# wooginawunan/multi-modal-uncertainty

Hardware: AMD Instinct MI355X
Metric: image+text samples/sec/node, MMBT Food-101 bs=256 seq=512; ECE/NLL parity (higher is better)
Workload: dtype bf16

## Files before the change

include/mmu.h:

```cpp
#ifndef MMU_H
#define MMU_H
#include <stdint.h>

#ifdef __cplusplus
extern "C" {
#endif

typedef void* mmu_stream_t;

enum { MMU_BF16 = 0, MMU_F32 = 1 };

#define MMU_ABI_VERSION 4
int mmu_version(void);
const char* mmu_last_error(void);

int mmu_set_seed_offset(const uint64_t* dev_counter);

int mmu_set_deterministic(int on);
int mmu_get_deterministic(void);

enum {
  MMU_EPI_STORE = 0,
  MMU_EPI_BIAS_GELU = 1,
  MMU_EPI_BIAS_DROP_RES = 2,
// ... 15 lines not shown
  int64_t ldx, aux_bstride;
  float* colsum;
  int64_t colsum_bstride;
  float drop_p;
  uint64_t seed;
  float* workspace;
  int64_t workspace_floats;
  const float* res_ln_mean;
  const float* res_ln_rstd;
  const float* res_ln_w;
  const float* res_ln_b;
  int64_t res_ln_bstride;
  const void* bn_x;
  const uint8_t* bn_mask;
  const float* bn_mean;
  const uint8_t* res_mask;
} mmu_epilogue;

int mmu_gemm(const void* A, int64_t lda, int a_kmajor,
             const void* B, int64_t ldb, int b_kmajor,
             void* C, int64_t ldc, int c_dtype,
             int64_t M, int64_t N, int64_t K,
             int64_t batch, int64_t strideA, int64_t strideB, int64_t strideC,
             const mmu_epilogue* epi, mmu_stream_t stream);

int mmu_gemm_rows(const void* A, int64_t lda, int a_kmajor,
                  const void* B, int64_t ldb, int b_kmajor,
                  void* C, int64_t ldc, int c_dtype,
                  int64_t M, int64_t N, int64_t K,
                  int64_t batch, int64_t strideA, int64_t strideB, int64_t strideC,
                  const mmu_epilogue* epi, int64_t drop_row_step, int64_t drop_row_offset,
                  mmu_stream_t stream);

int mmu_colsum_reduce(const float* partial, int64_t parts, int64_t N, float* out,
                      int accumulate, mmu_stream_t stream);
int mmu_colsum_reduce_multi(int n, const float* const* partial, const int64_t* parts, float* const* out, int64_t N,
                            int accumulate, mmu_stream_t stream);
int mmu_colsum_bf16(const void* X, int64_t M, int64_t N, int64_t ldx, float* partial,
                    float* out, int accumulate, mmu_stream_t stream);

int mmu_transpose_bf16_batched(const int64_t* jobs, int n_jobs, int64_t max_rows, int64_t max_cols,
                               mmu_stream_t stream);

int mmu_attention_fwd(const void* QKV, int64_t ld_qkv, const float* keymask,
                      void* O, int64_t ld_o, float* LSE,
                      int64_t batch, int64_t L, int64_t heads,
                      float drop_p, uint64_t seed, uint64_t* dropmask, mmu_stream_t stream);
int mmu_attention_bwd(const void* QKV, int64_t ld_qkv, const float* keymask,
                      const void* O, int64_t ld_o, const void* dO, int64_t ld_do,
                      const float* LSE, float* delta, void* dQKV, int64_t ld_dqkv,
                      int64_t batch, int64_t L, int64_t heads,
                      float drop_p, uint64_t seed, const uint64_t* dropmask, float* dbias_parts,
                      mmu_stream_t stream);

int mmu_attention_row0_fwd(const void* QKV, int64_t ld_qkv, const float* keymask,
                           void* O, int64_t ld_o, float* LSE,
                           int64_t batch, int64_t L, int64_t heads,
                           float drop_p, uint64_t seed, uint64_t* dropmask, mmu_stream_t stream);
int mmu_attention_row0_bwd(const void* QKV, int64_t ld_qkv, const float* keymask,
                           const void* O, int64_t ld_o, const void* dO, int64_t ld_do,
                           const float* LSE, void* dQKV, int64_t ld_dqkv,
                           int64_t batch, int64_t L, int64_t heads,
                           float drop_p, const uint64_t* dropmask, float* dbias_sums,
                           mmu_stream_t stream);

int mmu_layernorm_fwd(const void* X, const float* w, const float* b, void* Y,
// ... 184 lines not shown
```

multi-modal-uncertainty_amd/csrc/capi.hip:

```cpp
#include <stdarg.h>
#include <stdio.h>
#include <atomic>
#include <map>
#include <tuple>
#include <mutex>
#include <string>
#include <vector>
#include "mmu_internal.h"
#include <cstdlib>
#include <cmath>

using namespace mmu;

static thread_local std::string g_err;

namespace mmu {
const uint64_t* g_seed_off = nullptr;

static std::atomic<int> g_det{-1};
bool deterministic() {
  int v = g_det.load(std::memory_order_relaxed);
  if (v < 0) {
    const char* e = getenv("MMU_DETERMINISTIC");
    int want = (e && atoi(e) == 1) ? 1 : 0;
// ... 43 lines not shown

std::pair<hipEvent_t, hipEvent_t> take_events() {
  std::lock_guard<std::mutex> lk(g_t.mu);
  std::pair<hipEvent_t, hipEvent_t> ev;
  if (!g_t.pool.empty()) {
    ev = g_t.pool.back();
    g_t.pool.pop_back();
  } else {
    (void)hipEventCreate(&ev.first);
    (void)hipEventCreate(&ev.second);
  }
  return ev;
}
constexpr int64_t TAIL_WS_FLOATS = 8ll << 20;
float* tail_workspace(int64_t floats, hipStream_t s, int slot = 0) {
  static std::mutex mu;
  static std::map<std::tuple<int, hipStream_t, int>, float*> bufs;
  if (floats > TAIL_WS_FLOATS) return nullptr;
  int dev = 0;
  if (hipGetDevice(&dev) != hipSuccess) return nullptr;
  std::lock_guard<std::mutex> lk(mu);
  auto it = bufs.find({dev, s, slot});
  if (it != bufs.end()) return it->second;
  hipStreamCaptureStatus st = hipStreamCaptureStatusNone;
  if (hipStreamIsCapturing(s, &st) != hipSuccess || st != hipStreamCaptureStatusNone) return nullptr;
  void* b = nullptr;
  if (hipMalloc(&b, sizeof(float) * TAIL_WS_FLOATS) != hipSuccess) {
    (void)hipGetLastError();
    return nullptr;
  }
  bufs[{dev, s, slot}] = (float*)b;
  return (float*)b;
}
}

extern "C" {

int mmu_version(void) { return MMU_ABI_VERSION; }
const char* mmu_last_error(void) { return g_err.c_str(); }

int mmu_timing_enable(int on) {
  std::lock_guard<std::mutex> lk(g_t.mu);
  g_t.on = on != 0;
  for (auto& e : g_t.used) g_t.pool.push_back(e);
  g_t.used.clear();
  g_t.flops.clear();
  return 0;
}

int mmu_timing_pause(int paused) {
  std::lock_guard<std::mutex> lk(g_t.mu);
  g_t.paused = paused != 0;
  return 0;
}

int mmu_timing_read(double* total_ms, int64_t* launches, double* flops) {
  std::lock_guard<std::mutex> lk(g_t.mu);
  double tot = 0.0, fl = 0.0;
  for (size_t i = 0; i < g_t.used.size(); ++i) {
    (void)hipEventSynchronize(g_t.used[i].second);
    float ms = 0.f;
    if (hipEventElapsedTime(&ms, g_t.used[i].first, g_t.used[i].second) != hipSuccess) return fail("timing: elapsed");
    tot += ms;
    fl += g_t.flops[i];
  }
  *total_ms = tot;
  *launches = (int64_t)g_t.used.size();
  *flops = fl;
  return 0;
}

static int gemm_impl(const void* A, int64_t lda, int a_kmajor, const void* B, int64_t ldb, int b_kmajor, void* C,
                     int64_t ldc, int c_dtype, int64_t M, int64_t N, int64_t K, int64_t batch, int64_t strideA,
                     int64_t strideB, int64_t strideC, const mmu_epilogue* epi, int64_t drop_row_step,
                     int64_t drop_row_off, mmu_stream_t stream) {
  if (!A || !B || !C) return fail("mmu_gemm: null operand");
  if (M <= 0 || N <= 0 || K <= 0 || batch <= 0) return fail("mmu_gemm: bad shape M=%ld N=%ld K=%ld", M, N, K);
  if (N % 128) return fail("mmu_gemm: N=%ld must be a multiple of 128", N);
  if ((a_kmajor || b_kmajor) && K % 64) return fail("mmu_gemm: K=%ld must be a multiple of 64 for a K-major operand", K);
  if (!a_kmajor && M % 128) return fail("mmu_gemm: M=%ld must be a multiple of 128 when A is M-major", M);
  if ((lda % 8) || (ldb % 8) || (ldc % 4)) return fail("mmu_gemm: leading dims must be 16-B aligned");
  if (c_dtype != MMU_BF16 && c_dtype != MMU_F32) return fail("mmu_gemm: bad c_dtype");
  GemmParams p{};
  p.A = (const bf16*)A; p.B = (const bf16*)B; p.C = C;
  p.lda = lda; p.ldb = ldb; p.ldc = ldc; p.M = M; p.N = N; p.K = K;
  p.sA = strideA; p.sB = strideB; p.sC = strideC;
  p.drop_ldn = N * drop_row_step; p.drop_base = N * drop_row_off;
  const int64_t a_span = 2 * (a_kmajor ? (M + 256) * lda : (K + 64) * lda);
  const int64_t b_span = 2 * (b_kmajor ? (N + 256) * ldb : (K + 64) * ldb);
  const bool big = M >= 256 && N >= 256 && a_span < (1ll << 32) - 4096 && b_span < (1ll << 32) - 4096;
  const int tile = big ? 256 : 128;
  p.tiles_m = (int)((M + tile - 1) / tile);
  p.tiles_n = (int)((N + tile - 1) / tile);
  int kind = MMU_EPI_STORE;
  if (epi) kind = epi->kind;
  p.group_m = p.tiles_n <= 3 ? 1 : ((b_kmajor && kind != MMU_EPI_DGELU) ? 8 : 2);
  if (epi) {
    kind = epi->kind;
    p.accumulate = epi->accumulate;
    p.bias = epi->bias; p.bias_bstride = epi->bias_bstride;
    p.residual = epi->residual; p.ldr = epi->ldr; p.res_bstride = epi->res_bstride;
    p.aux = epi->aux; p.ldx = epi->ldx; p.aux_bstride = epi->aux_bstride;
    p.colsum = epi->colsum; p.colsum_bstride = epi->colsum_bstride;
    p.drop_p = epi->drop_p; p.seed = epi->seed; p.seed_off = g_seed_off;
    p.res_ln_mean = epi->res_ln_mean; p.res_ln_rstd = epi->res_ln_rstd;
    p.res_ln_w = epi->res_ln_w; p.res_ln_b = epi->res_ln_b; p.res_ln_bstride = epi->res_ln_bstride;
    p.bn_x = (const bf16*)epi->bn_x; p.bn_mask = epi->bn_mask; p.bn_mean = epi->bn_mean;
    p.res_mask = epi->res_mask;
  }
  p.kind = kind;
  if (kind < 0 || kind > MMU_EPI_ADD_RES_BNB) return fail("mmu_gemm: bad epilogue kind %d", kind);
  if ((kind == MMU_EPI_STORE_BNB || kind == MMU_EPI_ADD_RES_BNB) &&
      (!p.colsum || !p.bn_x || !p.bn_mean || batch != 1 || !a_kmajor || b_kmajor || p.accumulate || p.bias ||
       ldc != N || c_dtype != MMU_BF16))
    return fail("mmu_gemm: *_BNB needs the table (colsum), bn_x, bn_mean, batch 1, K-major A, N-major B, "
                "bf16 C with ldc == N, no bias / accumulate");
  if (kind == MMU_EPI_STORE_STATS && (!p.colsum || batch != 1 || !a_kmajor || !b_kmajor || p.accumulate))
    return fail("mmu_gemm: STORE_STATS needs the stats table (colsum), batch 1, K-major A and B, no accumulate");
  if (kind != MMU_EPI_STORE && kind != MMU_EPI_BIAS_DROP_RES && c_dtype != MMU_BF16)
    return fail("mmu_gemm: fused epilogues other than BIAS_DROP_RES write bf16");
  if (kind == MMU_EPI_BIAS_DROP_RES && c_dtype == MMU_F32 && (ldc % 4 || (epi && epi->ldr % 4)))
    return fail("mmu_gemm: f32 hidden-stream epilogue needs 16-B aligned rows");
  {
    const int nln = !!p.res_ln_mean + !!p.res_ln_rstd + !!p.res_ln_w + !!p.res_ln_b;
    if (nln && (nln != 4 || kind != MMU_EPI_BIAS_DROP_RES || c_dtype != MMU_F32))
      return fail("mmu_gemm: res_ln_* (all four) only with BIAS_DROP_RES into an f32 C");
  }
  if (kind == MMU_EPI_DGELU && !p.aux) return fail("mmu_gemm: DGELU epilogue needs aux");
  if ((kind == MMU_EPI_BIAS_DROP_RES || kind == MMU_EPI_ADD_RES || kind == MMU_EPI_ADD_RES_BNB) && !p.residual)
// ... 25 lines not shown
    if (p.res_ln_w && (off16(p.res_ln_w) || off16(p.res_ln_b) || (bat && p.res_ln_bstride % 4)))
      return fail("mmu_gemm: res_ln_w, res_ln_b and res_ln_bstride must keep 16-B alignment");
    if (p.res_ln_w && (((uintptr_t)p.res_ln_mean | (uintptr_t)p.res_ln_rstd) & 3))
      return fail("mmu_gemm: res_ln_mean / res_ln_rstd must be 4-B aligned");
    const bool table = kind == MMU_EPI_STORE_STATS || kind == MMU_EPI_STORE_BNB || kind == MMU_EPI_ADD_RES_BNB;
    if (table && off16(p.colsum)) return fail("mmu_gemm: the float2 table (colsum) must be 16-B aligned");
    if (!table && p.colsum && ((uintptr_t)p.colsum & 3)) return fail("mmu_gemm: colsum must be 4-B aligned");
    if (epi && epi->workspace && off16(epi->workspace))
      return fail("mmu_gemm: the split-K workspace must be 16-B aligned (float4 slabs)");
    if ((kind == MMU_EPI_STORE_BNB || kind == MMU_EPI_ADD_RES_BNB) && (off16(p.bn_x) || off16(p.bn_mean)))
      return fail("mmu_gemm: bn_x and bn_mean must be 16-B aligned");
  }
  p.splitk = 1;
  p.kchunk = K;
  if (kind == MMU_EPI_STORE && c_dtype == MMU_F32 && !p.bias && !p.colsum && epi && epi->workspace && K >= 1024) {
    const int64_t tiles = (int64_t)p.tiles_m * p.tiles_n * batch;
    const int64_t max_split = 64, min_k = K >= 32768 ? 1024 : 256;
    int64_t want = (640 + tiles - 1) / tiles;
    if (want > K / min_k) want = K / min_k;
    if (want > max_split) want = max_split;
    const int64_t cap = epi->workspace_floats / (batch * M * N);
    if (want > cap) want = cap;
    if (want >= 2) {
      int64_t chunk = (K + want - 1) / want;
      chunk = (chunk + 63) / 64 * 64;
      p.kchunk = chunk;
      p.splitk = (int)((K + chunk - 1) / chunk);
      p.ws = epi->workspace;
    }
  }
  const char* wide_env = getenv("MMU_GEMM_WIDE");
  const char* wide_min_env = getenv("MMU_GEMM_WIDE_MIN_TILES");
  const int wide_mode = wide_env ? atoi(wide_env) : 1;
  const int64_t wide_min = wide_min_env ? (int64_t)atoll(wide_min_env) : (int64_t)1024;
  const bool tail_kind = kind == MMU_EPI_STORE || kind == MMU_EPI_BIAS_GELU || kind == MMU_EPI_BIAS_DROP_RES ||
                         kind == MMU_EPI_DGELU || kind == MMU_EPI_ADD_RES;
  const bool wide_kind = tail_kind && kind != MMU_EPI_DGELU;
  const bool wide = (wide_mode == 2 ? tail_kind : wide_mode == 1 && wide_kind && N >= 2304) && big && a_kmajor &&
                    b_kmajor && N % 384 == 0 && p.splitk == 1 &&
                    2 * (M + 256) * lda < (1ll << 32) - 4096 && 2 * (N + 384) * ldb < (1ll << 32) - 4096 &&
                    (M + 255) / 256 * (N / 384) * batch >= wide_min;
  if (wide) {
    p.tiles_m = (int)((M + 255) / 256);
    p.tiles_n = (int)(N / 384);
    p.group_m = p.tiles_n <= 2 ? 1 : (kind != MMU_EPI_DGELU ? 8 : 2);
  }
  const char* tail_env = getenv("MMU_GEMM_TAIL");
  const int tail_mode = tail_env ? atoi(tail_env) : 1;
  int64_t tail_rows = 0, m_main = M, tail_chunk = K;
  int tail_split = 1;
  float* tail_ws = nullptr;
  if ((tail_mode == 2 || (tail_mode == 1 && wide)) && big && batch == 1 && p.splitk == 1 && tail_kind &&
      a_kmajor && K >= 512) {
    const int64_t tiles = (int64_t)p.tiles_m * p.tiles_n, left = tiles % 256;
    if (tiles > 256 && left > 0 && left % p.tiles_n == 0 && left * 8 <= 256) {
      m_main = (int64_t)(p.tiles_m - left / p.tiles_n) * 256;
      tail_rows = M - m_main;
      const int64_t st = (tail_rows + 127) / 128 * (N / 128);
      int64_t sk = 256 / st;
      if (sk > K / 256) sk = K / 256;
      if (sk < 1) sk = 1;
      tail_chunk = ((K + sk - 1) / sk + 63) / 64 * 64;
      tail_split = (int)((K + tail_chunk - 1) / tail_chunk);
      tail_ws = tail_split >= 2 ? tail_workspace((int64_t)tail_split * tail_rows * N, (hipStream_t)stream) : nullptr;
      if (!tail_ws) {
        tail_rows = 0;
        m_main = M;
      }
    }
  }
  hipStream_t s = (hipStream_t)stream;
  bool timed;
  std::pair<hipEvent_t, hipEvent_t> ev;
  {
    std::lock_guard<std::mutex> lk(g_t.mu);
    timed = g_t.on && !g_t.paused;
  }
  if (timed) {
    ev = take_events();
    (void)hipEventRecord(ev.first, s);
  }
  const bool det = deterministic();
  const char* csp_env = getenv("MMU_GEMM_CS_PART");
  const bool cs_plain = p.colsum && kind != MMU_EPI_STORE_STATS && kind != MMU_EPI_STORE_BNB &&
                        kind != MMU_EPI_ADD_RES_BNB;
  const bool cs_rows_ok = cs_plain && batch == 1 && p.splitk == 1 && (det || !csp_env || atoi(csp_env) != 0);
  const int cs_rows_main = (big && !wide) ? 128 : 64;
  const int64_t cs_parts_main = (m_main + cs_rows_main - 1) / cs_rows_main;
  const int64_t cs_parts = cs_parts_main + (tail_rows + 63) / 64;
  float* cs_part = cs_rows_ok ? tail_workspace(cs_parts * N, s, 1) : nullptr;
  if (det && cs_plain && !cs_part)
    return fail("mmu_gemm: deterministic mode: colsum with batch=%ld splitk=%d has no partial-row path%s",
// ... 824 lines not shown
```

multi-modal-uncertainty_amd/csrc/gemm.hip:

```cpp
#include "mmu_common.h"
#include "mmu_internal.h"
#include <cstdlib>
#include <type_traits>

namespace mmu {

constexpr int BKT = 64;
template <int N>
using ic = std::integral_constant<int, N>;

#ifdef MMU_GEMM_STAMPS
__device__ uint64_t g_gemm_stamps[1 << 16][4];
#define GEMM_STAMP(i)                                                                       \
  do {                                                                                      \
    if (threadIdx.x == 0) {                                                                 \
      const int lin_ = (int)(blockIdx.x + gridDim.x * (blockIdx.y + gridDim.y * blockIdx.z)); \
      if (lin_ < (1 << 16)) g_gemm_stamps[lin_][i] = __builtin_amdgcn_s_memtime();          \
    }                                                                                       \
  } while (0)
#else
#define GEMM_STAMP(i) \
  do {                \
  } while (0)
#endif
// ... 140 lines not shown
      d[r] = kz * fmaf(1.702f * u * sg, 1.0f - sg, sg);
    }
    if (xdst) {
      bf16x8 o;
#pragma unroll
      for (int r = 0; r < 8; ++r) o[r] = f2bf(d[r]);
      *(bf16x8*)xdst = o;
    }
  } else if (EPI == MMU_EPI_DGELU) {
#pragma unroll
    for (int r = 0; r < 8; ++r) v[r] *= in[r];
  } else if (EPI == MMU_EPI_ADD_RES) {
#pragma unroll
    for (int r = 0; r < 8; ++r) v[r] += in[r];
  }
  if (OUT_F32) {
    float4* C = (float4*)cdst;
    float4 lo = make_float4(v[0], v[1], v[2], v[3]), hi = make_float4(v[4], v[5], v[6], v[7]);
    if (p.accumulate) {
      const float4 c0 = C[0], c1 = C[1];
      lo.x += c0.x; lo.y += c0.y; lo.z += c0.z; lo.w += c0.w;
      hi.x += c1.x; hi.y += c1.y; hi.z += c1.z; hi.w += c1.w;
    }
    C[0] = lo;
    C[1] = hi;
  } else {
    bf16x8 o;
#pragma unroll
    for (int r = 0; r < 8; ++r) o[r] = f2bf(v[r]);
    *(bf16x8*)cdst = o;
  }
}

template <int EPI_, bool OUT_F32, int NJ, int PJ = 4>
static __device__ __forceinline__ void epilogue_block(const GemmParams& p, int64_t z, int slice, int64_t mw,
                                                      int64_t nw, f32x4 (&acc)[4][NJ], int l, char* ws) {
  constexpr bool BNB = EPI_ == MMU_EPI_STORE_BNB || EPI_ == MMU_EPI_ADD_RES_BNB;
  constexpr int EPI = EPI_ == MMU_EPI_STORE_BNB ? MMU_EPI_STORE : EPI_ == MMU_EPI_ADD_RES_BNB ? MMU_EPI_ADD_RES : EPI_;
  if (nw >= p.N) return;
  const int q = l & 7, rr = l >> 3;
  const int64_t n = nw + 8 * q;
  const bool slab = EPI == MMU_EPI_STORE && p.splitk > 1;
  float* slab_base = slab ? p.ws + (z * p.splitk + slice) * p.M * p.N : nullptr;
  const float* bias = (!slab && p.bias && EPI != MMU_EPI_DGELU && EPI != MMU_EPI_ADD_RES)
                          ? p.bias + z * p.bias_bstride : nullptr;
  const bf16* res = p.residual ? (const bf16*)p.residual + z * p.res_bstride : nullptr;
  bf16* aux = p.aux ? (bf16*)p.aux + z * p.aux_bstride : nullptr;
  const float scale = p.drop_p > 0.f ? 1.0f / (1.0f - p.drop_p) : 1.0f;
  const uint32_t thr = (uint32_t)(p.drop_p * 65536.0f + 0.5f);
  float bv[8];
  {
    float4 b0 = make_float4(0.f, 0.f, 0.f, 0.f), b1 = b0;
    if (bias) { b0 = *(const float4*)(bias + n); b1 = *(const float4*)(bias + n + 4); }
    bv[0] = b0.x; bv[1] = b0.y; bv[2] = b0.z; bv[3] = b0.w; bv[4] = b1.x; bv[5] = b1.y; bv[6] = b1.z; bv[7] = b1.w;
  }
  constexpr bool STATS = EPI == MMU_EPI_STORE_STATS;
  const bool want_cs = !STATS && !BNB && p.colsum != nullptr && !slab;
  constexpr bool TAB = STATS || BNB;
  float mu[8];
  const int64_t b_l = BNB ? (mw + rr) * p.N + n : 0;
  if (BNB) {
    const float4 m0 = *(const float4*)(p.bn_mean + n), m1 = *(const float4*)(p.bn_mean + n + 4);
    mu[0] = m0.x; mu[1] = m0.y; mu[2] = m0.z; mu[3] = m0.w; mu[4] = m1.x; mu[5] = m1.y; mu[6] = m1.z; mu[7] = m1.w;
  }
  float cs[8];
#pragma unroll
  for (int r = 0; r < 8; ++r) cs[r] = 0.f;
  constexpr bool LOADS = EPI == MMU_EPI_BIAS_DROP_RES || EPI == MMU_EPI_DGELU || EPI == MMU_EPI_ADD_RES;
  constexpr bool RES32 = OUT_F32 && EPI == MMU_EPI_BIAS_DROP_RES;
  const bf16* src = EPI == MMU_EPI_DGELU ? (const bf16*)aux : res;
  const float* src32 = RES32 && p.residual ? (const float*)p.residual + z * p.res_bstride : nullptr;
  const int64_t lds_ = EPI == MMU_EPI_DGELU ? p.ldx : p.ldr;
  const int64_t m_l = mw + rr;
  const int64_t in_l = m_l * lds_ + n;
  const int64_t c_l = z * p.sC + m_l * p.ldc + n;
  constexpr bool XST = EPI == MMU_EPI_BIAS_GELU || EPI == MMU_EPI_BIAS_DROP_QGELU;
  constexpr bool DRP = EPI == MMU_EPI_BIAS_DROP_RES || EPI == MMU_EPI_BIAS_DROP_QGELU;
  const int64_t x_l = XST ? m_l * p.ldx + n : 0;
  const int64_t s_l = EPI == MMU_EPI_STORE ? m_l * p.N + n : 0;
  const int64_t q_l = DRP ? p.drop_base + (z * p.M + m_l) * p.drop_ldn + n : 0;
  const uint64_t seed = DRP && thr ? mmu_eff_seed(p.seed, p.seed_off) : 0;
  const bool res_ln = RES32 && p.res_ln_w != nullptr && !slab;
  float lw[8], lb[8];
  if (RES32) {
    float4 w0 = make_float4(1.f, 1.f, 1.f, 1.f), w1 = w0, b0 = make_float4(0.f, 0.f, 0.f, 0.f), b1 = b0;
    if (res_ln) {
      const float* lw_ = p.res_ln_w + z * p.res_ln_bstride;
      const float* lb_ = p.res_ln_b + z * p.res_ln_bstride;
      w0 = *(const float4*)(lw_ + n); w1 = *(const float4*)(lw_ + n + 4);
      b0 = *(const float4*)(lb_ + n); b1 = *(const float4*)(lb_ + n + 4);
    }
    lw[0] = w0.x; lw[1] = w0.y; lw[2] = w0.z; lw[3] = w0.w; lw[4] = w1.x; lw[5] = w1.y; lw[6] = w1.z; lw[7] = w1.w;
    lb[0] = b0.x; lb[1] = b0.y; lb[2] = b0.z; lb[3] = b0.w; lb[4] = b1.x; lb[5] = b1.y; lb[6] = b1.z; lb[7] = b1.w;
  }
  static_assert(!TAB || PJ == 4, "STORE_STATS / *_BNB: one epilogue pass = one 64-row table block");
#pragma unroll
  for (int pass = 0; pass < NJ / PJ; ++pass) {
    float st1[8], st2[8];
    if (TAB) {
#pragma unroll
      for (int e = 0; e < 8; ++e) st1[e] = st2[e] = 0.f;
    }
    bf16x8 in[RES32 ? 1 : 2 * PJ];
    uint32_t rmk[EPI == MMU_EPI_ADD_RES ? 2 * PJ : 1];
    float4 in32[RES32 ? 2 * PJ : 1][2];
    float rmu[RES32 ? 2 * PJ : 1], rrs[RES32 ? 2 * PJ : 1];
#pragma unroll
    for (int it = 0; it < 2 * PJ; ++it) {
      const int d = 16 * PJ * pass + 8 * it;
      const int64_t m = m_l + d;
      if (RES32) {
        rmu[it] = 0.f;
        rrs[it] = 1.f;
        if (!slab && m < p.M) {
          const float* s32 = src32 + in_l + d * lds_;
          in32[it][0] = *(const float4*)s32;
          in32[it][1] = *(const float4*)(s32 + 4);
          if (res_ln) {
            rmu[it] = p.res_ln_mean[z * p.M + m];
            rrs[it] = p.res_ln_rstd[z * p.M + m];
          }
        } else {
          in32[it][0] = in32[it][1] = make_float4(0.f, 0.f, 0.f, 0.f);
        }
      } else if (LOADS && !slab && m < p.M) {
        in[it] = *(const bf16x8*)(src + in_l + d * lds_);
        if (EPI == MMU_EPI_ADD_RES) rmk[it] = p.res_mask ? (uint32_t)p.res_mask[(in_l + d * lds_) >> 3] : 0xFFu;
      } else {
        in[it] = bf16x8{};
        if (EPI == MMU_EPI_ADD_RES) rmk[it] = 0;
      }
    }
#pragma unroll
    for (int jj = 0; jj < PJ; ++jj) {
      const int r = 16 * jj + (l & 15);
#pragma unroll
      for (int i = 0; i < 4; ++i) {
        const int ch = 4 * i + (l >> 4);
        *(f32x4*)(ws + r * 256 + ((ch ^ (r & 15)) << 4)) = acc[i][PJ * pass + jj];
      }
    }
    bf16x8 bx[BNB ? 2 * PJ : 1];
    uint32_t bm[BNB ? 2 * PJ : 1];
    if (BNB) {
#pragma unroll
      for (int it = 0; it < 2 * PJ; ++it) {
        const int d = 16 * PJ * pass + 8 * it;
        if (!slab && m_l + d < p.M) {
          const int64_t o = b_l + (int64_t)d * p.N;
          bx[it] = *(const bf16x8*)(p.bn_x + o);
          bm[it] = p.bn_mask ? (uint32_t)p.bn_mask[o >> 3] : 0xFFu;
        } else {
          bx[it] = bf16x8{};
          bm[it] = 0;
        }
      }
    }
#pragma unroll
    for (int it = 0; it < 2 * PJ; ++it) {
      const int r = rr + 8 * it;
      const int d = 16 * PJ * pass + 8 * it;
      const int64_t m = m_l + d;
      const float4 lo = *(const float4*)(ws + r * 256 + (((2 * q) ^ (r & 15)) << 4));
      const float4 hi = *(const float4*)(ws + r * 256 + (((2 * q + 1) ^ (r & 15)) << 4));
      if (m >= p.M) continue;
      if (slab) {
        float4* sd = (float4*)(slab_base + s_l + d * p.N);
        sd[0] = lo;
        sd[1] = hi;
        continue;
      }
      float v[8] = {lo.x + bv[0], lo.y + bv[1], lo.z + bv[2], lo.w + bv[3],
                    hi.x + bv[4], hi.y + bv[5], hi.z + bv[6], hi.w + bv[7]};
      float inf[8];
      if (RES32) {
        inf[0] = in32[it][0].x; inf[1] = in32[it][0].y; inf[2] = in32[it][0].z; inf[3] = in32[it][0].w;
        inf[4] = in32[it][1].x; inf[5] = in32[it][1].y; inf[6] = in32[it][1].z; inf[7] = in32[it][1].w;
        if (res_ln) {
#pragma unroll
          for (int e = 0; e < 8; ++e) inf[e] = fmaf((inf[e] - rmu[it]) * rrs[it], lw[e], lb[e]);
        }
      } else {
#pragma unroll
        for (int r = 0; r < 8; ++r) inf[r] = LOADS ? bf2f(in[RES32 ? 0 : it][r]) : 0.f;
        if (EPI == MMU_EPI_ADD_RES) {
#pragma unroll
          for (int r = 0; r < 8; ++r) inf[r] = ((rmk[EPI == MMU_EPI_ADD_RES ? it : 0] >> r) & 1) ? inf[r] : 0.f;
        }
      }
      void* cdst = OUT_F32 ? (void*)((float*)p.C + c_l + d * p.ldc) : (void*)((bf16*)p.C + c_l + d * p.ldc);
      epi_oct<EPI, OUT_F32>(p, cdst, (XST && aux) ? aux + x_l + d * p.ldx : nullptr,
                            DRP ? (uint64_t)(q_l + d * p.drop_ldn) >> 2 : 0, v, inf, scale, thr, seed);
      if (want_cs) {
#pragma unroll
        for (int e = 0; e < 8; ++e) cs[e] += v[e];
      }
      if (STATS) {
#pragma unroll
        for (int e = 0; e < 8; ++e) {
          const float y = bf2f(f2bf(v[e]));
          st1[e] += y;
          st2[e] = fmaf(y, y, st2[e]);
        }
      }
      if (BNB) {
#pragma unroll
        for (int e = 0; e < 8; ++e) {
          const float g = ((bm[BNB ? it : 0] >> e) & 1) ? bf2f(f2bf(v[e])) : 0.f;
          st1[e] += g;
          st2[e] = fmaf(g, bf2f(bx[BNB ? it : 0][e]) - mu[e], st2[e]);
        }
      }
    }
    if (TAB) {
#pragma unroll
      for (int e = 0; e < 8; ++e) {
#pragma unroll
// ... 417 lines not shown
  dma_kmaj<6>(smem + W_TA, rb, p.ldb, n0, 0, w, l);
  asm volatile("s_waitcnt vmcnt(0)" ::: "memory");
  __syncthreads();
  for (int kt = 0; kt < nk; ++kt) {
    const char* sa = smem + (kt & 1) * W_STAGE;
    const char* sb = sa + W_TA;
    if (kt + 1 < nk) {
      char* d = smem + ((kt + 1) & 1) * W_STAGE;
      const int64_t k1 = (int64_t)(kt + 1) * BKT;
      dma_kmaj<4>(d, ra, p.lda, m0, k1, w, l);
      dma_kmaj<6>(d + W_TA, rb, p.ldb, n0, k1, w, l);
    }
#pragma unroll
    for (int ks = 0; ks < 2; ++ks) {
      bf16x8 fa[4];
#pragma unroll
      for (int j = 0; j < 4; ++j) fa[j] = s_frag<true, 512>(sa, 64 * wm + 16 * j, ks, l);
#pragma unroll
      for (int c = 0; c < 3; ++c) {
        bf16x8 fb[4];
#pragma unroll
        for (int i = 0; i < 4; ++i) fb[i] = s_frag<true, 512>(sb, 192 * wn + 64 * c + 16 * i, ks, l);
#pragma unroll
        for (int i = 0; i < 4; ++i)
#pragma unroll
          for (int j = 0; j < 4; ++j)
            acc[c][i][j] = __builtin_amdgcn_mfma_f32_16x16x32_bf16(fb[i], fa[j], acc[c][i][j], 0, 0, 0);
      }
    }
    asm volatile("s_waitcnt vmcnt(0)" ::: "memory");
    __syncthreads();
  }
  constexpr int PJ = (OUT_F32 && EPI == MMU_EPI_BIAS_DROP_RES) ? 1 : 2;
#pragma unroll
  for (int c = 0; c < 3; ++c)
    epilogue_block<EPI, OUT_F32, 4, PJ>(p, z, 0, m0 + 64 * wm, n0 + 192 * wn + 64 * c, acc[c], l, smem + w * 16384);
}

template <bool BNB>
__global__ __launch_bounds__(256) void splitk_reduce_tab_kernel(const GemmParams p) {
  __shared__ float red[4][2][8][8];
  const int t = threadIdx.x, oc = t & 7, rs = t >> 3, l = t & 63, w = t >> 6;
  const int64_t M = p.M, N = p.N, n = (int64_t)blockIdx.y * 64 + 8 * oc, r0 = (int64_t)blockIdx.x * 64;
  bf16* C = (bf16*)p.C;
  float a[8], b[8], mu[8];
#pragma unroll
  for (int e = 0; e < 8; ++e) a[e] = b[e] = mu[e] = 0.f;
  if (BNB) {
#pragma unroll
    for (int e = 0; e < 8; ++e) mu[e] = p.bn_mean[n + e];
  }
#pragma unroll
  for (int h = 0; h < 2; ++h) {
    const int64_t m = r0 + rs + 32 * h;
    if (m >= M) continue;
    const int64_t o = m * N + n;
    const float* sl = p.ws + o;
    float4 lo = *(const float4*)sl, hi = *(const float4*)(sl + 4);
    for (int k = 1; k < p.splitk; ++k) {
      const float4 c = *(const float4*)(sl + k * M * N), d = *(const float4*)(sl + k * M * N + 4);
      lo.x += c.x; lo.y += c.y; lo.z += c.z; lo.w += c.w;
      hi.x += d.x; hi.y += d.y; hi.z += d.z; hi.w += d.w;
    }
    const bf16x8 v = {f2bf(lo.x), f2bf(lo.y), f2bf(lo.z), f2bf(lo.w), f2bf(hi.x), f2bf(hi.y), f2bf(hi.z), f2bf(hi.w)};
    *(bf16x8*)(C + m * p.ldc + n) = v;
    if (BNB) {
      const bf16x8 x = *(const bf16x8*)(p.bn_x + o);
      const uint32_t mk = p.bn_mask ? (uint32_t)p.bn_mask[o >> 3] : 0xFFu;
#pragma unroll
// ... 477 lines not shown
```

multi-modal-uncertainty_amd/src/_native.py:

```python
import ctypes
import os

_HERE = os.path.dirname(os.path.abspath(__file__))
LIB_PATH = os.environ.get("MMU_LIB_PATH") or os.path.join(_HERE, "libmmu_hip.so")

c_i64, c_i32, c_f32, c_u64, c_vp = ctypes.c_int64, ctypes.c_int32, ctypes.c_float, ctypes.c_uint64, ctypes.c_void_p
c_f32p, c_i64p, c_dp = ctypes.POINTER(ctypes.c_float), ctypes.POINTER(ctypes.c_int64), ctypes.POINTER(ctypes.c_double)

MMU_BF16, MMU_F32 = 0, 1
(EPI_STORE, EPI_BIAS_GELU, EPI_BIAS_DROP_RES, EPI_DGELU, EPI_ADD_RES, EPI_BIAS_DROP_QGELU, EPI_STORE_STATS,
 EPI_STORE_BNB, EPI_ADD_RES_BNB) = range(9)


class Epilogue(ctypes.Structure):
    _fields_ = [("kind", c_i32), ("accumulate", c_i32), ("bias", c_vp), ("bias_bstride", c_i64),
                ("residual", c_vp), ("ldr", c_i64), ("res_bstride", c_i64), ("aux", c_vp), ("ldx", c_i64),
                ("aux_bstride", c_i64), ("colsum", c_vp), ("colsum_bstride", c_i64), ("drop_p", c_f32),
                ("seed", c_u64), ("workspace", c_vp), ("workspace_floats", c_i64), ("res_ln_mean", c_vp),
                ("res_ln_rstd", c_vp), ("res_ln_w", c_vp), ("res_ln_b", c_vp), ("res_ln_bstride", c_i64),
                ("bn_x", c_vp), ("bn_mask", c_vp), ("bn_mean", c_vp), ("res_mask", c_vp)]


SIGNATURES = {
    "mmu_version": (c_i32, []),
    "mmu_embed_bwd_ws_floats": (c_i64, [c_i64, c_i64, c_i64]),
    "mmu_embed_bwd_ws_floats_h": (c_i64, [c_i64, c_i64, c_i64, c_i64]),
    "mmu_last_error": (ctypes.c_char_p, []),
    "mmu_set_seed_offset": (c_i32, [c_vp]),
    "mmu_set_deterministic": (c_i32, [c_i32]),
    "mmu_get_deterministic": (c_i32, []),
    "mmu_embed_bwd_det_chunk": (c_i64, []),
    "mmu_gemm": (c_i32, [c_vp, c_i64, c_i32, c_vp, c_i64, c_i32, c_vp, c_i64, c_i32, c_i64, c_i64, c_i64,
                         c_i64, c_i64, c_i64, c_i64, ctypes.POINTER(Epilogue), c_vp]),
    "mmu_gemm_rows": (c_i32, [c_vp, c_i64, c_i32, c_vp, c_i64, c_i32, c_vp, c_i64, c_i32, c_i64, c_i64, c_i64,
                              c_i64, c_i64, c_i64, c_i64, ctypes.POINTER(Epilogue), c_i64, c_i64, c_vp]),
    "mmu_attention_row0_fwd": (c_i32, [c_vp, c_i64, c_vp, c_vp, c_i64, c_vp, c_i64, c_i64, c_i64, c_f32, c_u64, c_vp,
                                       c_vp]),
    "mmu_attention_row0_bwd": (c_i32, [c_vp, c_i64, c_vp, c_vp, c_i64, c_vp, c_i64, c_vp, c_vp, c_i64,
                                       c_i64, c_i64, c_i64, c_f32, c_vp, c_vp, c_vp]),
    "mmu_layernorm_bwd_f32_rows": (c_i32, [c_vp, c_vp, c_vp, c_vp, c_vp, c_vp, c_vp, c_f32, c_u64, c_vp, c_vp, c_vp,
                                           c_i64, c_i64, c_i64, c_i64, c_i64, c_vp]),
    "mmu_colsum_reduce": (c_i32, [c_vp, c_i64, c_i64, c_vp, c_i32, c_vp]),
    "mmu_colsum_reduce_multi": (c_i32, [c_i32, c_vp, c_vp, c_vp, c_i64, c_i32, c_vp]),
    "mmu_colsum_bf16": (c_i32, [c_vp, c_i64, c_i64, c_i64, c_vp, c_vp, c_i32, c_vp]),
    "mmu_transpose_bf16_batched": (c_i32, [c_vp, c_i32, c_i64, c_i64, c_vp]),
    "mmu_attention_fwd": (c_i32, [c_vp, c_i64, c_vp, c_vp, c_i64, c_vp, c_i64, c_i64, c_i64, c_f32, c_u64, c_vp,
                                  c_vp]),
    "mmu_attention_bwd": (c_i32, [c_vp, c_i64, c_vp, c_vp, c_i64, c_vp, c_i64, c_vp, c_vp, c_vp, c_i64,
                                  c_i64, c_i64, c_i64, c_f32, c_u64, c_vp, c_vp, c_vp]),
    "mmu_layernorm_fwd": (c_i32, [c_vp, c_vp, c_vp, c_vp, c_vp, c_vp, c_i64, c_i64, c_f32, c_i64, c_i64, c_vp]),
    "mmu_layernorm_bwd": (c_i32, [c_vp, c_vp, c_vp, c_vp, c_vp, c_vp, c_vp, c_f32, c_u64, c_vp, c_vp, c_vp,
                                  c_i64, c_i64, c_i64, c_vp]),
    "mmu_layernorm_fwd_f32": (c_i32, [c_vp, c_vp, c_vp, c_vp, c_vp, c_vp, c_vp, c_i64, c_i64, c_f32, c_i64, c_i64,
                                      c_vp]),
    "mmu_layernorm_bwd_f32": (c_i32, [c_vp, c_vp, c_vp, c_vp, c_vp, c_vp, c_vp, c_f32, c_u64, c_vp, c_vp, c_vp,
                                      c_i64, c_i64, c_i64, c_vp]),
    "mmu_layernorm_bwd_res": (c_i32, [c_vp, c_vp, c_vp, c_vp, c_vp, c_vp, c_vp, c_vp, c_vp, c_vp, c_i64, c_i64,
                                      c_i64, c_vp]),
    "mmu_seqattn_fwd": (c_i32, [c_vp, c_i64, c_vp, c_i64, c_vp, c_i64, c_i64, c_i64, c_i64, c_vp]),
    "mmu_seqattn_bwd": (c_i32, [c_vp, c_i64, c_vp, c_i64, c_vp, c_i64, c_vp, c_vp, c_vp, c_i64, c_i64, c_i64, c_i64,
                                c_i64, c_vp]),
    "mmu_embed_fwd": (c_i32, [c_vp, c_vp, c_vp, c_vp, c_vp, c_vp, c_vp, c_vp, c_vp, c_f32, c_i64, c_i64, c_vp,
                              c_i64, c_i64, c_i64, c_i64, c_i64, c_i64, c_f32, c_f32, c_u64, c_vp, c_vp, c_vp, c_vp,
                              c_vp, c_vp]),
    "mmu_embed_bwd": (c_i32, [c_vp, c_vp, c_vp, c_vp, c_vp, c_vp, c_vp, c_vp, c_vp, c_vp, c_i64, c_i64, c_i64,
                              c_i64, c_i64, c_i64, c_f32, c_f32, c_u64, c_vp, c_vp, c_vp, c_vp, c_vp, c_vp, c_vp,
                              c_vp]),
    "mmu_image_normalize": (c_i32, [c_vp, c_i64, c_f32p, c_f32p, c_vp, c_i32, c_vp]),
    "mmu_maxpool_fwd": (c_i32, [c_vp, c_i64, c_i64, c_i64, c_i64, c_vp, c_vp, c_vp]),
    "mmu_maxpool_bwd": (c_i32, [c_vp, c_vp, c_i64, c_i64, c_i64, c_i64, c_vp, c_vp]),
    "mmu_row_pool_fwd": (c_i32, [c_vp, c_i64, c_i64, c_i64, c_i64, c_i64, c_vp, c_vp]),
    "mmu_row_pool_bwd": (c_i32, [c_vp, c_i64, c_i64, c_i64, c_i64, c_i64, c_vp, c_vp]),
    "mmu_conv3x3_implicit": (c_i32, [c_vp, c_vp, c_vp, c_i64, c_i64, c_i64, c_i64, c_i64, c_vp, c_i64, c_vp]),
    "mmu_conv3x3_implicit_bnb": (c_i32, [c_vp, c_vp, c_vp, c_i64, c_i64, c_i64, c_i64, c_i64, c_vp, c_vp, c_vp,
# ... 28 lines not shown
                                  c_f32, c_f32, c_f32, c_f32, c_f32, c_f32, c_f32, c_vp, c_i64, c_vp]),
    "mmu_uncertainty": (c_i32, [c_vp, c_vp, c_i64, c_i64, c_i64, c_vp, c_vp, c_vp, c_vp, c_vp]),
    "mmu_ece_bins": (c_i32, [c_vp, c_vp, c_i64, c_i64, c_vp, c_vp]),
    "mmu_uncertainty_decompose": (c_i32, [c_vp, c_i64, c_i64, c_i64, c_vp, c_i64, c_i64, c_i64, c_i64, c_vp, c_vp,
                                          c_vp, c_vp]),
    "mmu_robustness_summary": (c_i32, [c_vp, c_i64, c_i64, c_i64, c_vp, c_i64, c_i64, c_i64, c_i64, c_vp, c_vp,
                                       c_vp]),
    "mmu_timing_enable": (c_i32, [c_i32]),
    "mmu_timing_pause": (c_i32, [c_i32]),
    "mmu_timing_read": (c_i32, [c_dp, c_i64p, c_dp]),
}

_lib = None


class NativeError(RuntimeError):
    pass


ABI_VERSION = 4


def load():
    global _lib
    if _lib is None:
        if not os.path.exists(LIB_PATH):
            raise NativeError(f"libmmu_hip.so not built at {LIB_PATH}: run `python -c 'import __graft_entry__ as g; "
                              f"g.build()'` (hipcc --offload-arch=gfx950)")
        import torch
        if torch.cuda.is_available():
            torch.cuda.init()
        lib = ctypes.CDLL(LIB_PATH)
        for name, (res, args) in SIGNATURES.items():
            fn = getattr(lib, name)
            fn.restype, fn.argtypes = res, args
        if lib.mmu_version() != ABI_VERSION:
            raise NativeError(f"libmmu_hip.so ABI {lib.mmu_version()} != {ABI_VERSION} (include/mmu.h "
                              "MMU_ABI_VERSION): rebuild the library")
        _lib = lib
    return _lib


def call(name, *args):
    rc = getattr(load(), name)(*args)
    if rc != 0:
        raise NativeError(f"{name}: {load().mmu_last_error().decode()}")
    return rc


def last_error():
    return load().mmu_last_error().decode()
```

Baseline: 1754.

## Prefetch DGELU aux rows across epilogue passes and derive GEMM thresholds from CU count

The DGELU epilogue now issues its aux-row loads one pass ahead, including across the three chained 64-column blocks of the wide kernel, using double-buffered registers. This overlaps global-load latency with the accumulator shuffling through shared memory. The wide-tile minimum and the tail split thresholds now come from the device CU count (one round = CU count, wide minimum = 4×CUs) instead of hard-coded 256 and 1024. Group-M selection is centralised with an env override and gives DGELU a larger group for wide tiles and K-major B. The extra prefetch buffers raise register pressure.

Measured after the change: 1757 (median of 3 runs). Within noise of the previous version (+0.2%).

```diff
diff --git a/include/mmu.h b/include/mmu.h
--- a/include/mmu.h
+++ b/include/mmu.h
@@ -71,6 +71,8 @@
                   const mmu_epilogue* epi, int64_t drop_row_step, int64_t drop_row_offset,
                   mmu_stream_t stream);
 
+int mmu_gemm_cu_thresholds(int cus, int64_t* round_tiles, int64_t* wide_min_tiles);
+
 int mmu_colsum_reduce(const float* partial, int64_t parts, int64_t N, float* out,
                       int accumulate, mmu_stream_t stream);
 int mmu_colsum_reduce_multi(int n, const float* const* partial, const int64_t* parts, float* const* out, int64_t N,
diff --git a/multi-modal-uncertainty_amd/csrc/capi.hip b/multi-modal-uncertainty_amd/csrc/capi.hip
--- a/multi-modal-uncertainty_amd/csrc/capi.hip
+++ b/multi-modal-uncertainty_amd/csrc/capi.hip
@@ -99,11 +99,49 @@
   bufs[{dev, s, slot}] = (float*)b;
   return (float*)b;
 }
+struct GemmCuPlan {
+  int64_t round, wide_min;
+};
+GemmCuPlan gemm_cu_plan(int cus) { return {(int64_t)cus, 4 * (int64_t)cus}; }
+
+int device_cus() {
+  static std::mutex mu;
+  static std::map<int, int> cus;
+  int dev = 0;
+  if (hipGetDevice(&dev) != hipSuccess) return 0;
+  std::lock_guard<std::mutex> lk(mu);
+  auto it = cus.find(dev);
+  if (it != cus.end()) return it->second;
+  hipDeviceProp_t prop;
+  if (hipGetDeviceProperties(&prop, dev) != hipSuccess) {
+    (void)hipGetLastError();
+    return 0;
+  }
+  cus[dev] = prop.multiProcessorCount;
+  return prop.multiProcessorCount;
+}
+
+int gemm_group_m(int tiles_n, bool wide, bool b_kmajor, int kind) {
+  const char* e = getenv("MMU_GEMM_GROUP_M");
+  if (e && atoi(e) >= 1) return atoi(e);
+  if (tiles_n <= (wide ? 2 : 3)) return 1;
+  if (kind == MMU_EPI_DGELU) return wide ? 8 : (b_kmajor ? 4 : 2);
+  return (wide || b_kmajor) ? 8 : 2;
+}
 }
 
 extern "C" {
 
 int mmu_version(void) { return MMU_ABI_VERSION; }
+
+int mmu_gemm_cu_thresholds(int cus, int64_t* round_tiles, int64_t* wide_min_tiles) {
+  if (cus < 0) cus = device_cus();
+  if (cus <= 0 || !round_tiles || !wide_min_tiles) return fail("mmu_gemm_cu_thresholds: no CU count / null output");
+  const GemmCuPlan cp = gemm_cu_plan(cus);
+  *round_tiles = cp.round;
+  *wide_min_tiles = cp.wide_min;
+  return 0;
+}
 const char* mmu_last_error(void) { return g_err.c_str(); }
 
 int mmu_timing_enable(int on) {
@@ -161,7 +199,7 @@
   p.tiles_n = (int)((N + tile - 1) / tile);
   int kind = MMU_EPI_STORE;
   if (epi) kind = epi->kind;
-  p.group_m = p.tiles_n <= 3 ? 1 : ((b_kmajor && kind != MMU_EPI_DGELU) ? 8 : 2);
+  p.group_m = gemm_group_m(p.tiles_n, false, b_kmajor != 0, kind);
   if (epi) {
     kind = epi->kind;
     p.accumulate = epi->accumulate;
@@ -253,7 +291,9 @@
   const char* wide_env = getenv("MMU_GEMM_WIDE");
   const char* wide_min_env = getenv("MMU_GEMM_WIDE_MIN_TILES");
   const int wide_mode = wide_env ? atoi(wide_env) : 1;
-  const int64_t wide_min = wide_min_env ? (int64_t)atoll(wide_min_env) : (int64_t)1024;
+  const GemmCuPlan cup = gemm_cu_plan(device_cus());
+  if (cup.round <= 0) return fail("mmu_gemm: no HIP device");
+  const int64_t wide_min = wide_min_env ? (int64_t)atoll(wide_min_env) : cup.wide_min;
   const bool tail_kind = kind == MMU_EPI_STORE || kind == MMU_EPI_BIAS_GELU || kind == MMU_EPI_BIAS_DROP_RES ||
                          kind == MMU_EPI_DGELU || kind == MMU_EPI_ADD_RES;
   const bool wide_kind = tail_kind && kind != MMU_EPI_DGELU;
@@ -264,7 +304,7 @@
   if (wide) {
     p.tiles_m = (int)((M + 255) / 256);
     p.tiles_n = (int)(N / 384);
-    p.group_m = p.tiles_n <= 2 ? 1 : (kind != MMU_EPI_DGELU ? 8 : 2);
+    p.group_m = gemm_group_m(p.tiles_n, true, true, kind);
   }
   const char* tail_env = getenv("MMU_GEMM_TAIL");
   const int tail_mode = tail_env ? atoi(tail_env) : 1;
@@ -273,12 +313,12 @@
   float* tail_ws = nullptr;
   if ((tail_mode == 2 || (tail_mode == 1 && wide)) && big && batch == 1 && p.splitk == 1 && tail_kind &&
       a_kmajor && K >= 512) {
-    const int64_t tiles = (int64_t)p.tiles_m * p.tiles_n, left = tiles % 256;
-    if (tiles > 256 && left > 0 && left % p.tiles_n == 0 && left * 8 <= 256) {
+    const int64_t tiles = (int64_t)p.tiles_m * p.tiles_n, left = tiles % cup.round;
+    if (tiles > cup.round && left > 0 && left % p.tiles_n == 0 && left * 8 <= cup.round) {
       m_main = (int64_t)(p.tiles_m - left / p.tiles_n) * 256;
       tail_rows = M - m_main;
       const int64_t st = (tail_rows + 127) / 128 * (N / 128);
-      int64_t sk = 256 / st;
+      int64_t sk = cup.round / st;
       if (sk > K / 256) sk = K / 256;
       if (sk < 1) sk = 1;
       tail_chunk = ((K + sk - 1) / sk + 63) / 64 * 64;
diff --git a/multi-modal-uncertainty_amd/csrc/gemm.hip b/multi-modal-uncertainty_amd/csrc/gemm.hip
--- a/multi-modal-uncertainty_amd/csrc/gemm.hip
+++ b/multi-modal-uncertainty_amd/csrc/gemm.hip
@@ -196,9 +196,25 @@
   }
 }
 
-template <int EPI_, bool OUT_F32, int NJ, int PJ = 4>
+template <int PJ>
+static __device__ __forceinline__ void dgelu_rows_request(const GemmParams& p, int64_t z, int64_t mw, int64_t nw,
+                                                          int pass, int l, bf16x8* in) {
+  const int q = l & 7, rr = l >> 3;
+  const bf16* src = (const bf16*)p.aux + z * p.aux_bstride;
+  const int64_t nb = nw < p.N ? nw : 0;
+  const int64_t m_l = mw + rr, in_l = m_l * p.ldx + nb + 8 * q;
+  const int64_t safe = (p.M - 1) * p.ldx + nb + 8 * q;
+#pragma unroll
+  for (int it = 0; it < 2 * PJ; ++it) {
+    const int d = 16 * PJ * pass + 8 * it;
+    in[it] = *(const bf16x8*)(src + (m_l + d < p.M ? in_l + d * p.ldx : safe));
+  }
+}
+
+template <int EPI_, bool OUT_F32, int NJ, int PJ = 4, int NEXT = 0>
 static __device__ __forceinline__ void epilogue_block(const GemmParams& p, int64_t z, int slice, int64_t mw,
-                                                      int64_t nw, f32x4 (&acc)[4][NJ], int l, char* ws) {
+                                                      int64_t nw, f32x4 (&acc)[4][NJ], int l, char* ws,
+                                                      bf16x8* pre = nullptr) {
   constexpr bool BNB = EPI_ == MMU_EPI_STORE_BNB || EPI_ == MMU_EPI_ADD_RES_BNB;
   constexpr int EPI = EPI_ == MMU_EPI_STORE_BNB ? MMU_EPI_STORE : EPI_ == MMU_EPI_ADD_RES_BNB ? MMU_EPI_ADD_RES : EPI_;
   if (nw >= p.N) return;
@@ -258,8 +274,14 @@
     lb[0] = b0.x; lb[1] = b0.y; lb[2] = b0.z; lb[3] = b0.w; lb[4] = b1.x; lb[5] = b1.y; lb[6] = b1.z; lb[7] = b1.w;
   }
   static_assert(!TAB || PJ == 4, "STORE_STATS / *_BNB: one epilogue pass = one 64-row table block");
-#pragma unroll
-  for (int pass = 0; pass < NJ / PJ; ++pass) {
+  constexpr bool AHEAD = EPI == MMU_EPI_DGELU;
+  constexpr int NPASS = NJ / PJ;
+  static_assert(NEXT == 0 || (AHEAD && NPASS % 2 == 0), "chained blocks: DGELU, an even number of passes");
+  bf16x8 own[AHEAD ? 2 : 1][AHEAD ? 2 * PJ : 1];
+  bf16x8* const rows[2] = {(AHEAD && pre) ? pre : own[0], own[AHEAD ? 1 : 0]};
+  if (AHEAD && !pre) dgelu_rows_request<PJ>(p, z, mw, nw, 0, l, rows[0]);
+#pragma unroll
+  for (int pass = 0; pass < NPASS; ++pass) {
     float st1[8], st2[8];
     if (TAB) {
 #pragma unroll
@@ -287,6 +309,7 @@
         } else {
           in32[it][0] = in32[it][1] = make_float4(0.f, 0.f, 0.f, 0.f);
         }
+      } else if (AHEAD) {
       } else if (LOADS && !slab && m < p.M) {
         in[it] = *(const bf16x8*)(src + in_l + d * lds_);
         if (EPI == MMU_EPI_ADD_RES) rmk[it] = p.res_mask ? (uint32_t)p.res_mask[(in_l + d * lds_) >> 3] : 0xFFu;
@@ -304,6 +327,11 @@
         *(f32x4*)(ws + r * 256 + ((ch ^ (r & 15)) << 4)) = acc[i][PJ * pass + jj];
       }
     }
+    if (AHEAD) {
+      if (pass + 1 < NPASS) dgelu_rows_request<PJ>(p, z, mw, nw, pass + 1, l, rows[(pass + 1) & 1]);
+      else if (NEXT > 0) dgelu_rows_request<PJ>(p, z, mw, nw + NEXT, 0, l, rows[0]);
+    }
+    const bf16x8* cur = AHEAD ? rows[pass & 1] : in;
     bf16x8 bx[BNB ? 2 * PJ : 1];
     uint32_t bm[BNB ? 2 * PJ : 1];
     if (BNB) {
@@ -346,7 +374,7 @@
         }
       } else {
 #pragma unroll
-        for (int r = 0; r < 8; ++r) inf[r] = LOADS ? bf2f(in[RES32 ? 0 : it][r]) : 0.f;
+        for (int r = 0; r < 8; ++r) inf[r] = LOADS ? bf2f(cur[RES32 ? 0 : it][r]) : 0.f;
         if (EPI == MMU_EPI_ADD_RES) {
 #pragma unroll
           for (int r = 0; r < 8; ++r) inf[r] = ((rmk[EPI == MMU_EPI_ADD_RES ? it : 0] >> r) & 1) ? inf[r] : 0.f;
@@ -830,9 +858,18 @@
     __syncthreads();
   }
   constexpr int PJ = (OUT_F32 && EPI == MMU_EPI_BIAS_DROP_RES) ? 1 : 2;
-#pragma unroll
-  for (int c = 0; c < 3; ++c)
-    epilogue_block<EPI, OUT_F32, 4, PJ>(p, z, 0, m0 + 64 * wm, n0 + 192 * wn + 64 * c, acc[c], l, smem + w * 16384);
+  if constexpr (EPI == MMU_EPI_DGELU) {
+    bf16x8 pre[2 * PJ];
+    dgelu_rows_request<PJ>(p, z, m0 + 64 * wm, n0 + 192 * wn, 0, l, pre);
+    char* ws = smem + w * 16384;
+    epilogue_block<EPI, OUT_F32, 4, PJ, 64>(p, z, 0, m0 + 64 * wm, n0 + 192 * wn, acc[0], l, ws, pre);
+    epilogue_block<EPI, OUT_F32, 4, PJ, 64>(p, z, 0, m0 + 64 * wm, n0 + 192 * wn + 64, acc[1], l, ws, pre);
+    epilogue_block<EPI, OUT_F32, 4, PJ, 0>(p, z, 0, m0 + 64 * wm, n0 + 192 * wn + 128, acc[2], l, ws, pre);
+  } else {
+#pragma unroll
+    for (int c = 0; c < 3; ++c)
+      epilogue_block<EPI, OUT_F32, 4, PJ>(p, z, 0, m0 + 64 * wm, n0 + 192 * wn + 64 * c, acc[c], l, smem + w * 16384);
+  }
 }
 
 template <bool BNB>
diff --git a/multi-modal-uncertainty_amd/src/_native.py b/multi-modal-uncertainty_amd/src/_native.py
--- a/multi-modal-uncertainty_amd/src/_native.py
+++ b/multi-modal-uncertainty_amd/src/_native.py
@@ -40,6 +40,7 @@
                                        c_i64, c_i64, c_i64, c_f32, c_vp, c_vp, c_vp]),
     "mmu_layernorm_bwd_f32_rows": (c_i32, [c_vp, c_vp, c_vp, c_vp, c_vp, c_vp, c_vp, c_f32, c_u64, c_vp, c_vp, c_vp,
                                            c_i64, c_i64, c_i64, c_i64, c_i64, c_vp]),
+    "mmu_gemm_cu_thresholds": (c_i32, [c_i32, c_i64p, c_i64p]),
     "mmu_colsum_reduce": (c_i32, [c_vp, c_i64, c_i64, c_vp, c_i32, c_vp]),
     "mmu_colsum_reduce_multi": (c_i32, [c_i32, c_vp, c_vp, c_vp, c_i64, c_i32, c_vp]),
     "mmu_colsum_bf16": (c_i32, [c_vp, c_i64, c_i64, c_i64, c_vp, c_vp, c_i32, c_vp]),
@@ -134,7 +135,12 @@
             torch.cuda.init()
         lib = ctypes.CDLL(LIB_PATH)
         for name, (res, args) in SIGNATURES.items():
-            fn = getattr(lib, name)
+            try:
+                fn = getattr(lib, name)
+            except AttributeError:
+                if not os.environ.get("MMU_LIB_PATH"):
+                    raise
+                continue
             fn.restype, fn.argtypes = res, args
         if lib.mmu_version() != ABI_VERSION:
             raise NativeError(f"libmmu_hip.so ABI {lib.mmu_version()} != {ABI_VERSION} (include/mmu.h "
```
